# ZJU-FAST-Lab/uneven_planner

Measured on AMD Instinct MI355X. Metric: MINCO traj-opts/sec (batch), higher is better.
Workload: dtype f64

## Files before the change

### include/uneven_hip.h

```cpp
#ifndef UNEVEN_HIP_H
#define UNEVEN_HIP_H

#include <stdint.h>

#ifdef __cplusplus
extern "C" {
#endif

typedef struct uph_map uph_map;
typedef struct uph_ctx uph_ctx;
typedef struct uph_kino uph_kino;

#define UPH_OK 0
#define UPH_ERR_INVALID (-1)
#define UPH_ERR_HIP (-2)
#define UPH_ERR_NO_DEVICE (-3)
#define UPH_ERR_LIMIT (-4)
#define UPH_ERR_NO_CACHE (-5)

#define UPH_RET_STOPPED 3
#define UPH_RET_UNSUPPORTED 4

#define UPH_RET_LEFT_TILE 5
#define UPH_TILE_MARGIN 2.0
// ... 174 lines not shown
int uph_kino_stats(uph_kino* k, double* kernel_ms);

#define UPH_PLAN_PATH_CAP 1024
int uph_plan_upload(uph_kino* k, uph_ctx* c, const uph_manager_params* mp, int32_t B, const double* starts, const double* goals, int32_t path_cap,
                    int32_t* status, int32_t* traj_of, int32_t* n_inner_xy, int32_t* n_inner_yaw);
int uph_replan_upload(uph_kino* k, uph_ctx* src, uph_ctx* dst, const uph_manager_params* mp, int32_t B, const int32_t* src_traj, const double* t_switch,
                      const double* goals, int32_t path_cap, double* switch_states, int32_t* status, int32_t* traj_of, int32_t* n_inner_xy, int32_t* n_inner_yaw);
int uph_traj_states(uph_ctx* c, int32_t n, const int32_t* traj, const double* t, double* out10);
#define UPH_REFINE_AT_END 7
int uph_refine_upload(uph_ctx* src, uph_ctx* dst, int32_t B, const int32_t* src_traj, const double* t_switch, double* switch_states ,
                      int32_t* status, int32_t* traj_of, int32_t* n_inner_xy, int32_t* n_inner_yaw);
int uph_plan_staged(uph_ctx* c, int32_t cap_xy, int32_t cap_yaw, double* init_xy, double* end_xy, double* init_yaw, double* end_yaw, double* inner_xy,
                    double* inner_yaw, int32_t* n_inner_xy, int32_t* n_inner_yaw, double* total_time);

int uph_ctx_create(uph_map* m, const uph_opt_params* p, uph_ctx** out);
void uph_ctx_destroy(uph_ctx* c);
int uph_ctx_set_lanes(uph_ctx* c, int32_t lanes);
int uph_ctx_set_xcd_locality(uph_ctx* c, int32_t group);
int uph_ctx_set_wps(uph_ctx* c, int32_t wps);
int uph_ctx_set_sample_precision(uph_ctx* c, int32_t bits);
int uph_ctx_set_rho(uph_ctx* c, double rho);
int uph_ctx_get_rho(uph_ctx* c, double* rho);
int uph_ctx_set_trial_abandon(uph_ctx* c, int32_t on);

int uph_ctx_set_trace(uph_ctx* c, int32_t cap);
int uph_ctx_get_trace(uph_ctx* c, double* out);

int uph_optimize_batch(uph_ctx* c, int32_t B, const uph_problem* probs, uph_result* results);
int uph_optimize_batch_multi(uph_ctx* const* ctxs, int32_t n_gpus, int32_t B, const uph_problem* probs, uph_result* results);
int uph_multi_batch_plan(int32_t n_gpus, int32_t B, const uph_problem* probs, int32_t* share_of, double* predicted_cost);
int uph_batch_count(const uph_ctx* c);
int uph_batch_origin(const uph_ctx* c, int32_t* idx);
int uph_batch_upload(uph_ctx* c, int32_t B, const uph_problem* probs);
int uph_batch_solve(uph_ctx* c);
int uph_batch_solve_async(uph_ctx* c);
int uph_batch_wait(uph_ctx* c);
int uph_batch_download(uph_ctx* c, uph_result* results);
int uph_batch_stats(uph_ctx* c, double* kernel_ms, int64_t* evals, int64_t* sample_evals, int64_t* lbfgs_iters, int64_t* hist_bytes);
int uph_batch_abandon_stats(uph_ctx* c, int64_t* out5);

int uph_batch_prepare_ms(uph_ctx* c, double* ms);

int uph_batch_cycles(uph_ctx* c, long long* out);

int uph_eval_batch(uph_ctx* c, const double* x_packed, double* f, double* grad_packed, int32_t repeat);
int uph_penalty_batch(uph_ctx* c, int32_t repeat, int32_t store_residuals, double* cost, double* gdcxy_packed, double* gdcyaw_packed, double* gdT2);
// ... 67 lines not shown
```

### uneven_planner_amd/_lib.py

```python
import ctypes as C
import os

_HERE = os.path.dirname(os.path.abspath(__file__))
LIB_PATH = os.environ.get("UNEVENHIP_LIB") or os.path.join(_HERE, "libunevenhip.so")


class MapParams(C.Structure):
    _fields_ = [("iter_num", C.c_int32), ("map_size_x", C.c_double), ("map_size_y", C.c_double),
                ("ellipsoid_x", C.c_double), ("ellipsoid_y", C.c_double), ("ellipsoid_z", C.c_double),
                ("xy_resolution", C.c_double), ("yaw_resolution", C.c_double), ("min_cnormal", C.c_double),
                ("max_rho", C.c_double), ("gravity", C.c_double)]


class OptParams(C.Structure):
    _fields_ = [("rho_T", C.c_double), ("rho_ter", C.c_double), ("max_vel", C.c_double), ("max_acc_lon", C.c_double),
                ("max_acc_lat", C.c_double), ("max_kap", C.c_double), ("min_cxi", C.c_double), ("max_sig", C.c_double),
                ("use_scaling", C.c_int32), ("rho", C.c_double), ("beta", C.c_double), ("gamma", C.c_double),
                ("epsilon_con", C.c_double), ("max_iter", C.c_double), ("g_epsilon", C.c_double),
                ("min_step", C.c_double), ("inner_max_iter", C.c_double), ("delta", C.c_double),
                ("mem_size", C.c_int32), ("past", C.c_int32), ("int_K", C.c_int32)]


class ManagerParams(C.Structure):
    _fields_ = [("piece_len", C.c_double), ("mean_vel", C.c_double), ("init_time_times", C.c_double), ("yaw_piece_times", C.c_double),
# ... 78 lines not shown
    "uph_batch_count": (C.c_int, [_VP]),
    "uph_batch_origin": (C.c_int, [_VP, C.POINTER(_I32)]),
    "uph_map_cells_device": (C.c_int, [_VP, C.POINTER(_VP), C.POINTER(_I64)]),
    "uph_map_commit": (C.c_int, [_VP]),
    "uph_map_export_slab_dev": (C.c_int, [_VP, _I32, _I32, _VP]),
    "uph_map_import_cells_dev": (C.c_int, [_VP, _VP]),
    "uph_terrain_query": (C.c_int, [_VP, DP, _I32, DP, DP]),
    "uph_frontend_query": (C.c_int, [_VP, DP, _I32, DP, C.POINTER(C.c_int32), C.POINTER(C.c_int32)]),
    "uph_terrain_pose_query": (C.c_int, [_VP, DP, _I32, DP]),
    "uph_frontend_query_ms": (C.c_int, [_VP, DP]),
    "uph_map_filter_cloud": (_I64, [C.POINTER(C.c_float), _I64, C.POINTER(C.c_float), _I64]),
    "uph_map_build_stats": (C.c_int, [_VP, DP, C.POINTER(_I64), C.POINTER(_I64)]),
    "uph_map_build_stages": (C.c_int, [_VP, DP]),
    "uph_map_built_cloud": (_I64, [_VP, C.POINTER(C.c_float), _I64]),
    "uph_ctx_create": (C.c_int, [_VP, C.POINTER(OptParams), C.POINTER(_VP)]),
    "uph_ctx_destroy": (None, [_VP]),
    "uph_ctx_set_lanes": (C.c_int, [_VP, _I32]),
    "uph_ctx_set_wps": (C.c_int, [_VP, _I32]),
    "uph_ctx_set_xcd_locality": (C.c_int, [_VP, _I32]),
    "uph_ctx_set_sample_precision": (C.c_int, [_VP, _I32]),
    "uph_ctx_set_rho": (C.c_int, [_VP, C.c_double]),
    "uph_ctx_get_rho": (C.c_int, [_VP, DP]),
    "uph_ctx_set_trial_abandon": (C.c_int, [_VP, _I32]),
    "uph_ctx_set_trace": (C.c_int, [_VP, _I32]),
    "uph_ctx_get_trace": (C.c_int, [_VP, DP]),
    "uph_optimize_batch": (C.c_int, [_VP, _I32, C.POINTER(Problem), C.POINTER(Result)]),
    "uph_batch_upload": (C.c_int, [_VP, _I32, C.POINTER(Problem)]),
    "uph_batch_solve": (C.c_int, [_VP]),
    "uph_batch_solve_async": (C.c_int, [_VP]),
    "uph_batch_wait": (C.c_int, [_VP]),
    "uph_batch_download": (C.c_int, [_VP, C.POINTER(Result)]),
    "uph_batch_stats": (C.c_int, [_VP, DP, C.POINTER(_I64), C.POINTER(_I64), C.POINTER(_I64), C.POINTER(_I64)]),
    "uph_batch_prepare_ms": (C.c_int, [_VP, DP]),
    "uph_batch_abandon_stats": (C.c_int, [_VP, C.POINTER(_I64)]),
    "uph_batch_cycles": (C.c_int, [_VP, C.POINTER(C.c_longlong)]),
    "uph_build_id": (C.c_char_p, []),
    "uph_eval_batch": (C.c_int, [_VP, DP, DP, DP, _I32]),
    "uph_penalty_batch": (C.c_int, [_VP, _I32, _I32, DP, DP, DP, DP]),
    "uph_init_scaling_batch": (C.c_int, [_VP]),
    "uph_microbench_batch": (C.c_int, [_VP, _I32]),
    "uph_batch_set_state": (C.c_int, [_VP, DP, DP, DP, DP, DP]),
    "uph_report_batch": (C.c_int, [_VP, DP]),
    "uph_rollout_sizes": (C.c_int, [_I32, C.POINTER(_I32), DP, C.POINTER(_I32), DP, C.c_double, _I32, C.POINTER(_I64)]),
    "uph_rollout_plan": (C.c_int, [_VP, C.c_double, _I32, C.POINTER(_I64)]),
    "uph_rollout_batch": (C.c_int, [_VP, C.c_double, _I32, _I32, _I32, _I32, DP]),
    "uph_rollout_batch_dev": (C.c_int, [_VP, C.c_double, _I32, _I32, _I32, _I32, _VP]),
# ... 120 lines not shown
```

### uneven_planner_amd/alm_traj_opt.py

```python
import ctypes as C

import numpy as np

from . import _lib

HILL_OPT_PARAMS = dict(rho_T=100000.0, rho_ter=10.0, max_vel=0.5, max_acc_lon=5.0, max_acc_lat=10.0, max_kap=2.1,
                       min_cxi=0.8, max_sig=0.05, use_scaling=True, rho=1.0, beta=1000.0, gamma=1.0,
                       epsilon_con=0.001, max_iter=10.0, g_epsilon=1.0e-3, min_step=1.0e-32, inner_max_iter=10000.0,
                       delta=1.0e-4, mem_size=256, past=3, int_K=16)
_INT_FIELDS = ("use_scaling", "mem_size", "past", "int_K")


def pack_problems(probs, int_K=16, with_sizes=False):
    arr = (_lib.Problem * len(probs))()
    keep, sizes = [], []
    for i, pr in enumerate(probs):
        ixy = np.ascontiguousarray(np.asarray(pr["inner_xy"], dtype=np.float64).T)
        iyw = np.ascontiguousarray(pr["inner_yaw"], dtype=np.float64)
        keep += [ixy, iyw]
        a = arr[i]
        a.n_inner_xy, a.n_inner_yaw = ixy.shape[0], iyw.shape[0]
        a.init_xy[:] = np.asarray(pr["init_xy"], dtype=np.float64).T.ravel().tolist()
        a.end_xy[:] = np.asarray(pr["end_xy"], dtype=np.float64).T.ravel().tolist()
        a.init_yaw[:] = np.asarray(pr["init_yaw"], dtype=np.float64).ravel().tolist()
# ... 411 lines not shown
            self.h = None
        p = _lib.OptParams(**{k: (int(getattr(self, k)) if k in _INT_FIELDS else float(getattr(self, k))) for k in self._pnames})
        h = C.c_void_p()
        _lib.check(self.L.uph_ctx_create(env.h, C.byref(p), C.byref(h)), "uph_ctx_create")
        self.h = h

    def set_lanes(self, lanes):
        _lib.check(self.L.uph_ctx_set_lanes(self.h, int(lanes)), "uph_ctx_set_lanes")

    def set_xcd_locality(self, group):
        _lib.check(self.L.uph_ctx_set_xcd_locality(self.h, int(group)), "uph_ctx_set_xcd_locality")

    def set_wps(self, wps):
        _lib.check(self.L.uph_ctx_set_wps(self.h, int(wps)), "uph_ctx_set_wps")

    def set_sample_precision(self, bits):
        _lib.check(self.L.uph_ctx_set_sample_precision(self.h, int(bits)), "uph_ctx_set_sample_precision")

    def set_rho(self, rho):
        _lib.check(self.L.uph_ctx_set_rho(self.h, float(rho)), "uph_ctx_set_rho")

    def set_trial_abandon(self, on):
        _lib.check(self.L.uph_ctx_set_trial_abandon(self.h, 1 if on else 0), "uph_ctx_set_trial_abandon")

    def get_rho(self):
        r = C.c_double(0)
        _lib.check(self.L.uph_ctx_get_rho(self.h, C.byref(r)), "uph_ctx_get_rho")
        return r.value

    def _make_problems(self, probs):
        arr, keep, self._sizes = pack_problems(probs, int(self.int_K), with_sizes=True)
        return arr, keep

    def upload(self, probs):
        arr, keep = self._make_problems(probs)
        self._B = 0
        _lib.check(self.L.uph_batch_upload(self.h, len(probs), arr), "uph_batch_upload")
        self._B = len(probs)
        self._trace_cap_up = getattr(self, "_trace_cap", 0)

    def solve(self):
        _lib.check(self.L.uph_batch_solve(self.h), "uph_batch_solve")

    def solve_async(self):
        _lib.check(self.L.uph_batch_solve_async(self.h), "uph_batch_solve_async")

# ... 529 lines not shown
```

### uneven_planner_amd/csrc/solver_program.hpp

```cpp
#pragma once
#include "terrain_dev.hpp"
#include "trajectory_dev.hpp"
#include "uph_common.hpp"

namespace uph {

#ifndef UPH_GRID_FROM_MEM
#define UPH_GRID_FROM_MEM 1
#endif
#ifndef UPH_PHASE_MASK
#define UPH_PHASE_MASK 15
#endif
#ifndef UPH_STATE_PROBE
#define UPH_STATE_PROBE(st) do { } while (0)
#endif
#ifndef UPH_SCALING_WB
#define UPH_SCALING_WB 8
#endif
#ifndef UPH_SC_XB
#define UPH_SC_XB 9
#endif
#ifndef UPH_SC_YB
#define UPH_SC_YB 14
#endif
#ifndef UPH_SC_WLO
#define UPH_SC_WLO 2
#endif
#ifndef UPH_SC_WHI
#define UPH_SC_WHI 3
#endif

#ifndef UPH_ASIDE_PREP
#define UPH_ASIDE_PREP 1
#endif
template <class WG, class F>
UPH_HD void asideKnotSolve(WG& wg, int lenW, int lenX, int n, F f) {
    (void)lenW; (void)lenX;
    wg.pfor(n, f);
}

template <class WG, class SR = double>
struct Solver {
    WG& wg;
    const GridDev& grid;
    const OptParams& P;
    const BatchDev& bd;
    const TrajDesc& td;
    int Nxy, Nyaw, n, S, K, mem, CH, CHP, recd;
    int CHS;
    int* rtag;
    double *x, *xp, *g, *gp, *d, *cxy, *cyaw, *Gxy, *Gyaw, *gamxy, *gamyaw, *bt, *rec, *wtab, *ttab, *pf, *hd;
    double* ab;
    int* abn;
    static constexpr int AB_DOUBLES = 4;
    double* up;
    static constexpr int UP_DOUBLES = 6;
    UPH_HD void tally(int k, bool yes) {
#if defined(__HIP_DEVICE_COMPILE__)
        if (yes && wg.wave == 0) abn[k] = abn[k] + 1;
#else
        if (yes) abn[k]++;
#endif
// ... 802 lines not shown

    UPH_HD void initScaling(double* x0) {
        generate<false>(x0, 0.0);
        const double tau = x0[0];
        const double dTau = getTtoTauGrad(tau);
        double js[3];
        expand(x0, 1.0, js);
        double sm[3] = {0.0, 0.0, 0.0};
        for (int s0 = 0; s0 < S; s0 += CHS) {
            const int cnt = S - s0 < CHS ? S - s0 : CHS;
            double part[3];
            wg.template sum<3>(cnt, part, [&](int t, double* acc) { sampleObjective(s0 + t, t, acc); });
            sm[0] += part[0]; sm[1] += part[1]; sm[2] += part[2];
            scatterChunk(s0, cnt);
        }
        double chx, chy;
        adjoint(chx, chy);
        const double gTau_fx = (P.rho_T + (js[1] + sm[1] + chx) / Nxy + (js[2] + sm[2] + chy) / Nyaw) * dTau;
        const double mq = wg.maxv((Nxy - 1) * 2 + (Nyaw - 1), [&](int t) {
            return t < (Nxy - 1) * 2 ? fabs(gamxy[3 * 2 + t]) : fabs(gamyaw[3 + (t - (Nxy - 1) * 2)]);
        });
        scale_fx = wg.bcast(1.0 / dmax(1.0, dmax(mq, fabs(gTau_fx))));
        wg.pfor(2, [&](int u) { fillTimes(u); });
        wg.pfor(S, [&](int s) { scalingSample(s, dTau); });
    }

    UPH_HD void scalingSample(int s, double dTau) {
        const int i = divSmall(s, K + 1, inv_k1), j = s - i * (K + 1);
        Kin k;
        kin(i, j, k);
#if !defined(UPH_SCALING_GROUPS) || UPH_SCALING_GROUPS == 2
        scalingGroup<0, 4>(s, i, j, k, dTau);
        scalingGroup<4, 3>(s, i, j, k, dTau);
#elif UPH_SCALING_GROUPS == 3
        scalingGroup<0, 3>(s, i, j, k, dTau);
        scalingGroup<3, 2>(s, i, j, k, dTau);
        scalingGroup<5, 2>(s, i, j, k, dTau);
#else
        scalingGroup<0, 7>(s, i, j, k, dTau);
#endif
    }
    template <int Q0, int NQS>
    UPH_HD void scalingGroup(int s, int i, int j, const Kin& k, double dTau) {
        const int nbx = Nxy + 5, nby = Nyaw + 5;
        const double Tx = Txy, Ty = Tyaw, itx = 1.0 / Txy, ity = 1.0 / Tyaw;
        const double gravity = grid.gravity;
        const double alpha = 1.0 / K * j;
        const double icvx = k.tv[0], icvy = k.tv[2], icxi = k.tv[5];
        const int m = k.yaw_idx;
        double dpL[NQS][2], dvL[NQS][2], daL[NQS][2], dpR[NQS][2], dvR[NQS][2], daR[NQS][2];
        double ypL[NQS], yvL[NQS], yaL[NQS], ypR[NQS], yvR[NQS], yaR[NQS];
        double sumx[NQS], sumy[NQS], mx[NQS];
#pragma unroll
        for (int qi = 0; qi < NQS; qi++) {
            const int q = Q0 + qi;
            double gp_[2] = {0, 0}, gv_[2] = {0, 0}, ga_[2] = {0, 0}, gyaw = 0.0, gdyaw = 0.0, gse2[3];
            if (q == 0) {
                gv_[0] = k.syaw; gv_[1] = -k.cyaw;
                gyaw = k.vel[0] * k.cyaw + k.vel[1] * k.syaw;
            } else if (q == 1) {
                for (int t = 0; t < 2; t++) gv_[t] = 1.0 * icvx * icvx * 2.0 * k.vel[t];
                for (int t = 0; t < 3; t++) gse2[t] = 1.0 * k.v_norm * k.v_norm * 2.0 * icvx * k.tg[0][t];
                gp_[0] = gse2[0]; gp_[1] = gse2[1]; gyaw = gse2[2];
            } else if (q == 2) {
                const double gax = 2.0 * k.ax;
                ga_[0] = gax * icvx * k.cyaw; ga_[1] = gax * icvx * k.syaw;
                gyaw = gax * icvx * k.lat_acc;
// ... 31 lines not shown
                chain_y += -(double)kk * cyaw[6 * m + kk] * ity * vy;
                gy_[kk] = vy * sy;
                sx *= itx; sy *= ity;
            }
            double tx = ((gp_[0] * k.vel[0] + gp_[1] * k.vel[1]) + (gv_[0] * k.acc[0] + gv_[1] * k.acc[1]) + (ga_[0] * k.jer[0] + ga_[1] * k.jer[1])) * alpha;
            const double yawdot = gyaw * k.dyaw + gdyaw * k.d2yaw;
            tx += yawdot * (alpha + i);
            const double ty = -yawdot * m;
            sumx[qi] = tx + chain_x;
            sumy[qi] = ty + chain_y;
            mx[qi] = 0.0;
            for (int t = 0; t < 2; t++) {
                const double g0 = gx_[0][t], g1 = gx_[1][t], g2 = gx_[2][t], g3 = gx_[3][t], g4 = gx_[4][t], g5 = gx_[5][t];
                dpL[qi][t] = g0 - 10.0 * g3 + 15.0 * g4 - 6.0 * g5; dvL[qi][t] = g1 - 6.0 * g3 + 8.0 * g4 - 3.0 * g5; daL[qi][t] = 0.5 * g2 - 1.5 * g3 + 1.5 * g4 - 0.5 * g5;
                dpR[qi][t] = 10.0 * g3 - 15.0 * g4 + 6.0 * g5; dvR[qi][t] = -4.0 * g3 + 7.0 * g4 - 3.0 * g5; daR[qi][t] = 0.5 * g3 - g4 + 0.5 * g5;
            }
            {
                const double g0 = gy_[0], g1 = gy_[1], g2 = gy_[2], g3 = gy_[3], g4 = gy_[4], g5 = gy_[5];
                ypL[qi] = g0 - 10.0 * g3 + 15.0 * g4 - 6.0 * g5; yvL[qi] = g1 - 6.0 * g3 + 8.0 * g4 - 3.0 * g5; yaL[qi] = 0.5 * g2 - 1.5 * g3 + 1.5 * g4 - 0.5 * g5;
                ypR[qi] = 10.0 * g3 - 15.0 * g4 + 6.0 * g5; yvR[qi] = -4.0 * g3 + 7.0 * g4 - 3.0 * g5; yaR[qi] = 0.5 * g3 - g4 + 0.5 * g5;
            }
        }
        const bool inL = i >= 1, inR = i + 1 <= Nxy - 1;
        const auto WL = UPH_AS_GLOBAL(Wr_xy + (size_t)(inL ? 2 * (i - 1) : 0) * nbx);
        const auto WR = UPH_AS_GLOBAL(Wr_xy + (size_t)(inR ? 2 * i : 0) * nbx);
        const int pcL = knotCol(i, Nxy), pcR = knotCol(i + 1, Nxy);
        for (int c0 = 3; c0 < Nxy + 2; c0 += UPH_SCALING_WB) {
            double w[4][UPH_SCALING_WB];
#pragma unroll
            for (int u = 0; u < UPH_SCALING_WB; u++) {
                const int cc = c0 + u < Nxy + 2 ? c0 + u : Nxy + 1;
                w[0][u] = WL[cc]; w[1][u] = WL[nbx + cc]; w[2][u] = WR[cc]; w[3][u] = WR[nbx + cc];
            }
#pragma unroll
            for (int q = 0; q < NQS; q++) {
                const double c00 = inL ? dvL[q][0] : 0.0, c01 = inL ? dvL[q][1] : 0.0, c10 = inL ? daL[q][0] : 0.0, c11 = inL ? daL[q][1] : 0.0;
                const double c20 = inR ? dvR[q][0] : 0.0, c21 = inR ? dvR[q][1] : 0.0, c30 = inR ? daR[q][0] : 0.0, c31 = inR ? daR[q][1] : 0.0;
                double mq = mx[q];
#pragma unroll
                for (int u = 0; u < UPH_SCALING_WB; u++) {
                    const int col = c0 + u;
                    double a0 = (w[0][u] * c00 + w[1][u] * c10) + (w[2][u] * c20 + w[3][u] * c30);
                    double a1 = (w[0][u] * c01 + w[1][u] * c11) + (w[2][u] * c21 + w[3][u] * c31);
                    if (col == pcL) { a0 += dpL[q][0]; a1 += dpL[q][1]; }
                    if (col == pcR) { a0 += dpR[q][0]; a1 += dpR[q][1]; }
                    if (col < Nxy + 2) mq = dmax(mq, dmax(fabs(a0), fabs(a1)));
                }
                mx[q] = mq;
            }
        }
        double htx[NQS], hty[NQS];
        {
            const int sc[4] = {1, 2, Nxy + 3, Nxy + 4};
            double w[4][4];
#pragma unroll
            for (int u = 0; u < 4; u++) { w[0][u] = WL[sc[u]]; w[1][u] = WL[nbx + sc[u]]; w[2][u] = WR[sc[u]]; w[3][u] = WR[nbx + sc[u]]; }
#pragma unroll
            for (int q = 0; q < NQS; q++) {
                const double c00 = inL ? dvL[q][0] : 0.0, c01 = inL ? dvL[q][1] : 0.0, c10 = inL ? daL[q][0] : 0.0, c11 = inL ? daL[q][1] : 0.0;
                const double c20 = inR ? dvR[q][0] : 0.0, c21 = inR ? dvR[q][1] : 0.0, c30 = inR ? daR[q][0] : 0.0, c31 = inR ? daR[q][1] : 0.0;
                double a0[4], a1[4];
#pragma unroll
                for (int u = 0; u < 4; u++) {
                    a0[u] = (w[0][u] * c00 + w[1][u] * c10) + (w[2][u] * c20 + w[3][u] * c30);
                    a1[u] = (w[0][u] * c01 + w[1][u] * c11) + (w[2][u] * c21 + w[3][u] * c31);
                }
                if (!inL) { a0[0] += dvL[q][0]; a1[0] += dvL[q][1]; a0[1] += daL[q][0]; a1[1] += daL[q][1]; }
                if (!inR) { a0[2] += dvR[q][0]; a1[2] += dvR[q][1]; a0[3] += daR[q][0]; a1[3] += daR[q][1]; }
                double headtail_x = 0.0;
                headtail_x += a0[0] * hd[2] + a1[0] * hd[3];
                headtail_x += 2.0 * Tx * (a0[1] * hd[4] + a1[1] * hd[5]);
                headtail_x += a0[2] * hd[8] + a1[2] * hd[9];
                headtail_x += 2.0 * Tx * (a0[3] * hd[10] + a1[3] * hd[11]);
                htx[q] = headtail_x;
            }
        }
        const bool yL = m >= 1, yR = m + 1 <= Nyaw - 1;
        const auto VL = UPH_AS_GLOBAL(Wr_yaw + (size_t)(yL ? 2 * (m - 1) : 0) * nby);
        const auto VR = UPH_AS_GLOBAL(Wr_yaw + (size_t)(yR ? 2 * m : 0) * nby);
        const int qL = knotCol(m, Nyaw), qR = knotCol(m + 1, Nyaw);
        for (int c0 = 3; c0 < Nyaw + 2; c0 += UPH_SCALING_WB) {
            double w[4][UPH_SCALING_WB];
#pragma unroll
            for (int u = 0; u < UPH_SCALING_WB; u++) {
                const int cc = c0 + u < Nyaw + 2 ? c0 + u : Nyaw + 1;
                w[0][u] = VL[cc]; w[1][u] = VL[nby + cc]; w[2][u] = VR[cc]; w[3][u] = VR[nby + cc];
            }
#pragma unroll
            for (int q = 0; q < NQS; q++) {
                const double y0_ = yL ? yvL[q] : 0.0, y1_ = yL ? yaL[q] : 0.0, y2_ = yR ? yvR[q] : 0.0, y3_ = yR ? yaR[q] : 0.0;
                double mq = mx[q];
#pragma unroll
                for (int u = 0; u < UPH_SCALING_WB; u++) {
                    const int col = c0 + u;
                    double a0 = (w[0][u] * y0_ + w[1][u] * y1_) + (w[2][u] * y2_ + w[3][u] * y3_);
                    if (col == qL) a0 += ypL[q];
                    if (col == qR) a0 += ypR[q];
                    if (col < Nyaw + 2) mq = dmax(mq, fabs(a0));
                }
                mx[q] = mq;
            }
        }
        {
            const int sc[4] = {1, 2, Nyaw + 3, Nyaw + 4};
            double w[4][4];
#pragma unroll
            for (int u = 0; u < 4; u++) { w[0][u] = VL[sc[u]]; w[1][u] = VL[nby + sc[u]]; w[2][u] = VR[sc[u]]; w[3][u] = VR[nby + sc[u]]; }
#pragma unroll
            for (int q = 0; q < NQS; q++) {
                const double y0_ = yL ? yvL[q] : 0.0, y1_ = yL ? yaL[q] : 0.0, y2_ = yR ? yvR[q] : 0.0, y3_ = yR ? yaR[q] : 0.0;
                double a0[4];
#pragma unroll
                for (int u = 0; u < 4; u++) a0[u] = (w[0][u] * y0_ + w[1][u] * y1_) + (w[2][u] * y2_ + w[3][u] * y3_);
                if (!yL) { a0[0] += yvL[q]; a0[1] += yaL[q]; }
                if (!yR) { a0[2] += yvR[q]; a0[3] += yaR[q]; }
                double headtail_y = 0.0;
// ... 453 lines not shown
```

### uneven_planner_amd/csrc/unevenhip.hip

```cpp
#include <hip/hip_runtime.h>

#include <type_traits>

#include <algorithm>
#include <cmath>
#include <cstdio>
#include <cstdlib>
#include <cstring>
#include <map>
#include <numeric>
#include <string>
#include <thread>
#include <vector>

#include "../../include/uneven_hip.h"
#include "minco_op_host.hpp"
#include "resample_walk.hpp"
#include "solver_program.hpp"
#include "uph_ctx.hpp"
#include "wave_dev.hpp"

using namespace uph;

#ifndef UPH_THOMAS_KPL
// ... 453 lines not shown
            else twoLoopT<8, 2>(d, g, dg_out, al_lds, n, hist, m, end, bound, scale);
            __builtin_amdgcn_s_setprio(0);
        }
        bar(1);
    }
    template <class F>
    __device__ __forceinline__ double maxv(int n, F f) {
        double a = 0.0;
        for (int i = ftid(); i < n; i += NT) { const double v = f(i); a = v > a ? v : a; }
        a = waveMax(a);
        double* r = red + par * (NW * MAXM);
        par ^= 1;
        if (lane == 0) r[wave * MAXM] = a;
        bar(0);
        double t = r[0];
#pragma unroll
        for (int w = 1; w < NW; w++) t = r[w * MAXM] > t ? r[w * MAXM] : t;
        return uni(t);
    }
};

template <int NT, class F>
__device__ __forceinline__ void asideKnotSolve(DevWG<NT>& wg, int lenW, int lenX, int n, F f) { wg.aside(lenW, lenX, n, f); }

template <int NT, int WPS, int MODE, bool F32S = false>
__global__ __launch_bounds__(NT, WPS) void uph_solver_kernel(GridDev grid, OptParams P, BatchDev bd, int repeat) {
    extern __shared__ double lds[];
    const int w = blockIdx.x;
    if (w >= bd.B) return;
    const int b = bd.order ? bd.order[w] : w;
    DevWG<NT> wg(lds);
    typedef typename std::conditional<F32S, f32r, double>::type SR;
    Solver<DevWG<NT>, SR> sol(wg, grid, P, bd, b, lds + DevWG<NT>::SCRATCH);
    TrajState& st = bd.state[b];
    if (MODE == 0) sol.evalOnly(st, repeat);
    else if (MODE == 1) sol.prepare(st);
    else if (MODE == 2) sol.optimize(st, repeat);
    else if (MODE == 7) sol.resumeHook(st, repeat >> 1, repeat & 1);
    else if (MODE == 8) { if (repeat & 1) sol.template penaltyOnly<true>(st, repeat >> 1); else sol.template penaltyOnly<false>(st, repeat >> 1); }
    else if (MODE == 3) sol.report(st);
    else if (MODE == 5) sol.microbench(st, repeat);
    else sol.scalingOnly(st);
}

__global__ void uph_fill_kernel(double* __restrict__ p, size_t n, double v) {
    for (size_t i = (size_t)blockIdx.x * blockDim.x + threadIdx.x; i < n; i += (size_t)gridDim.x * blockDim.x) p[i] = v;
// ... 218 lines not shown
            HIPCHK(hipMemcpyAsync(c->d_gridmem.p, c->grid_host_framed.data(), sizeof(GridDev) * c->frames.size(), hipMemcpyHostToDevice, c->stream));
            c->framed_from = grid;
            c->framed_valid = true;
        }
    }
    return UPH_OK;
}

int refreshStates(uph_ctx* c) {
    HIPCHK(hipMemcpy(c->state_host.data(), c->d_state.p, sizeof(TrajState) * c->B, hipMemcpyDeviceToHost));
    return UPH_OK;
}

static int launchSolver(uph_ctx* c, int mode, int repeat, bool async = false, hipEvent_t evb = nullptr, hipEvent_t eve = nullptr) {
    if (!async && c->pending) { setError("an asynchronous solve is in flight on this context: call uph_batch_wait first"); return UPH_ERR_INVALID; }
    if (!evb) { evb = c->ev0; eve = c->ev1; }
    HIPCHK(hipSetDevice(uphMapDevice(c->map)));
    GridDev grid;
    const int rg = syncGridMem(c, grid);
    if (rg != UPH_OK) return rg;
    if (c->d_parammem.ensure(sizeof(OptParams))) return UPH_ERR_HIP;
    HIPCHK(hipMemcpyAsync(c->d_parammem.p, &c->P, sizeof(OptParams), hipMemcpyHostToDevice, c->stream));
    BatchDev bd = makeBatchDev(c);
#define UPH_LAUNCH(NTL, WPS, MODE)                                                                                                     \
    do {                                                                                                                             \
        const size_t ldsmax = 160 * 1024;    \
        HIPCHK(hipFuncSetAttribute((const void*)uph_solver_kernel<NTL, WPS, MODE>, hipFuncAttributeMaxDynamicSharedMemorySize, (int)ldsmax)); \
        HIPCHK(hipEventRecord(evb, c->stream));                                                                                   \
        BatchDev bm = bd;                                                                                                            \
        bm.B = c->n_main;                                                                                                            \
        if (c->n_main < c->B) {            \
            BatchDev bb = bd;              \
            bb.B = c->B - c->n_main;                                                                                                 \
            bb.order = bd.order + c->n_main;                                                                                         \
            HIPCHK(hipStreamWaitEvent(c->stream2, evb, 0));                                                                       \
            hipLaunchKernelGGL((uph_solver_kernel<NTL, WPS, MODE>), dim3(bb.B), dim3(NTL), c->lds_big, c->stream2, grid, c->P, bb, repeat); \
            HIPCHK(hipEventRecord(c->ev2, c->stream2));                                                                              \
        }                                                                                                                            \
        hipLaunchKernelGGL((uph_solver_kernel<NTL, WPS, MODE>), dim3(c->n_main), dim3(NTL), c->lds_bytes, c->stream, grid, c->P, bm, repeat); \
        if (c->n_main < c->B) HIPCHK(hipStreamWaitEvent(c->stream, c->ev2, 0));                                                      \
    } while (0)
#define UPH_LAUNCH_MODE(NTL, WPS)                                                                                                      \
    do {                                                                                                                             \
        if (mode == 0) UPH_LAUNCH(NTL, WPS, 0);                                                                                      \
        else if (mode == 1) UPH_LAUNCH(NTL, WPS, 1);                                                                                 \
        else if (mode == 2) UPH_LAUNCH(NTL, WPS, 2);                                                                                 \
        else if (mode == 3) UPH_LAUNCH(NTL, WPS, 3);                                                                                 \
        else if (mode == 5) UPH_LAUNCH(NTL, WPS, 5);                                                                                 \
        else UPH_LAUNCH(NTL, WPS, 4);                                                                                                \
    } while (0)
#define UPH_LAUNCH32(NTL, WPS, MODE)                                                                                                   \
    do {                                                                                                                             \
        const size_t ldsmax = 160 * 1024;    \
        HIPCHK(hipFuncSetAttribute((const void*)uph_solver_kernel<NTL, WPS, MODE, true>, hipFuncAttributeMaxDynamicSharedMemorySize, (int)ldsmax)); \
        HIPCHK(hipEventRecord(evb, c->stream));                                                                                   \
        BatchDev bm = bd;                                                                                                            \
        bm.B = c->n_main;                                                                                                            \
        if (c->n_main < c->B) {                                                                                                      \
            BatchDev bb = bd;                                                                                                        \
            bb.B = c->B - c->n_main;                                                                                                 \
            bb.order = bd.order + c->n_main;                                                                                         \
            HIPCHK(hipStreamWaitEvent(c->stream2, evb, 0));                                                                       \
// ... 119 lines not shown
    if (c->ev0) hipEventDestroy(c->ev0);
    if (c->ev1) hipEventDestroy(c->ev1);
    if (c->stream) hipStreamDestroy(c->stream);
    if (c->stream2) hipStreamDestroy(c->stream2);
    if (c->ev2) hipEventDestroy(c->ev2);
    if (c->evp0) hipEventDestroy(c->evp0);
    if (c->evp1) hipEventDestroy(c->evp1);
    delete c;
}

int uph_ctx_set_lanes(uph_ctx* c, int32_t lanes) {
    if (!c || (lanes != 0 && lanes != 64 && lanes != 128 && lanes != 256 && lanes != 512)) return UPH_ERR_INVALID;
    c->lanes_forced = lanes;
    return UPH_OK;
}
int uph_ctx_set_xcd_locality(uph_ctx* c, int32_t group) { if (!c || group < 0) return UPH_ERR_INVALID; c->xcd_group = group; return UPH_OK; }
int uph_ctx_set_wps(uph_ctx* c, int32_t wps) { if (!c || wps < 0 || wps > 2) return UPH_ERR_INVALID; c->wps_forced = wps; return UPH_OK; }
int uph_ctx_set_sample_precision(uph_ctx* c, int32_t bits) {
    if (!c || (bits != 32 && bits != 64)) { setError("uph_ctx_set_sample_precision: 32 or 64"); return UPH_ERR_INVALID; }
    c->sample_f32 = bits == 32;
    return UPH_OK;
}
int uph_ctx_set_rho(uph_ctx* c, double rho) { if (!c) return UPH_ERR_INVALID; c->rho = rho; return UPH_OK; }
int uph_ctx_set_trial_abandon(uph_ctx* c, int32_t on) { if (!c || (on != 0 && on != 1)) return UPH_ERR_INVALID; c->P.no_trial_abandon = on ? 0 : 1; return UPH_OK; }
int uph_ctx_get_rho(uph_ctx* c, double* rho) { if (!c || !rho) return UPH_ERR_INVALID; *rho = c->rho; return UPH_OK; }

int uph_ctx_set_trace(uph_ctx* c, int32_t cap) { if (!c || cap < 0) return UPH_ERR_INVALID; c->trace_cap = cap; return UPH_OK; }
int uph_ctx_get_trace(uph_ctx* c, double* out ) {
    if (c && c->pending) { setError("an asynchronous solve is in flight on this context: call uph_batch_wait first"); return UPH_ERR_INVALID; }
    if (!c || !out || c->trace_cap_up <= 0 || c->B <= 0) return UPH_ERR_INVALID;
    HIPCHK(hipSetDevice(uphMapDevice(c->map)));
    HIPCHK(hipMemcpy(out, c->d_trace.p, sizeof(double) * (size_t)c->B * c->trace_cap_up, hipMemcpyDeviceToHost));
    return UPH_OK;
}

static void yawTurnKink(const uph_problem& pr, double& turn, double& kink) {
    double prev = pr.init_yaw[0];
    turn = 0.0; kink = 0.0;
    for (int i = 0; i <= pr.n_inner_yaw; i++) {
        const double cur = i < pr.n_inner_yaw ? pr.inner_yaw[i] : pr.end_yaw[0];
        const double dy = std::fabs(cur - prev);
        turn += dy; kink = std::max(kink, dy); prev = cur;
    }
}
static double predictedCostOf(int32_t n_inner_xy, int32_t n_inner_yaw, double turn, double kink) {
    const double n = 2.0 * n_inner_xy + n_inner_yaw + 1.0;
// ... 139 lines not shown
            const int G = c->xcd_group & ~7;
            for (int g0 = 0; g0 + G <= B; g0 += G) {
                std::vector<int> bins[8], spill, placed((size_t)G, -1);
                for (int k = 0; k < G; k++) bins[octant(c->order[g0 + k])].push_back(c->order[g0 + k]);
                for (int r = 0; r < 8; r++) {
                    int at = r;
                    for (int b : bins[r]) { if (at < G) { placed[at] = b; at += 8; } else spill.push_back(b); }
                }
                size_t sp = 0;
                for (int k = 0; k < G; k++) if (placed[k] < 0) placed[k] = spill[sp++];
                for (int k = 0; k < G; k++) c->order[g0 + k] = placed[k];
            }
        }
        const size_t limit = c->lanes == 128 ? 40960 : (c->lanes == 256 ? 81920 : (c->lanes == 512 ? 163840 : 32768));
        c->n_main = B; c->lds_big = 0;
        size_t mmain = 0, mbig = 0;
        int nbig = 0;
        for (int b = 0; b < B; b++) { if (c->fp_bytes[b] > limit) { nbig++; mbig = std::max(mbig, c->fp_bytes[b]); } else mmain = std::max(mmain, c->fp_bytes[b]); }
        if (nbig > 0 && nbig < B) {
            std::stable_partition(c->order.begin(), c->order.end(), [&](int a) { return c->fp_bytes[a] <= limit; });
            c->n_main = B - nbig; c->lds_bytes = mmain; c->lds_big = mbig;
        }
    }
    c->state_host.assign(B, TrajState());
    for (int b = 0; b < B; b++) { std::memset(&c->state_host[b], 0, sizeof(TrajState)); c->state_host[b].rho = c->rho; c->state_host[b].scale_fx = 1.0; }
    return UPH_OK;
}

static int commitBatch(uph_ctx* c, int32_t B) {
    HIPCHK(hipMemcpyAsync(c->d_desc.p, c->desc.data(), sizeof(TrajDesc) * B, hipMemcpyHostToDevice, c->stream));
    HIPCHK(hipMemcpyAsync(c->d_order.p, c->order.data(), 4 * B, hipMemcpyHostToDevice, c->stream));
    HIPCHK(hipMemcpyAsync(c->d_state.p, c->state_host.data(), sizeof(TrajState) * B, hipMemcpyHostToDevice, c->stream));
    HIPCHK(hipMemsetAsync(c->d_hist.p, 0, 8 * c->sum_hist, c->stream));
    HIPCHK(hipMemsetAsync(c->d_dual.p, 0, 8 * 7 * c->sum_S, c->stream));
    HIPCHK(hipMemsetAsync(c->d_res.p, 0, 8 * 7 * c->sum_S, c->stream));
    hipLaunchKernelGGL(uph_fill_kernel, dim3(1024), dim3(256), 0, c->stream, c->d_scl.as<double>(), (size_t)7 * c->sum_S, 1.0);
    HIPCHK(hipGetLastError());
    if (c->trace_cap > 0) HIPCHK(hipMemsetAsync(c->d_trace.p, 0, 8 * (size_t)c->trace_cap * B, c->stream));
    HIPCHK(hipStreamSynchronize(c->stream));
    c->trace_cap_up = c->trace_cap;
    c->B = B;
    return UPH_OK;
}

int uph_batch_upload(uph_ctx* c, int32_t B, const uph_problem* probs) {
    if (!c || B <= 0 || !probs) { setError("uph_batch_upload: bad arguments"); return UPH_ERR_INVALID; }
// ... 736 lines not shown
```

### uneven_planner_amd/csrc/uph_common.hpp

```cpp
#pragma once
#include <math.h>
#include <stdint.h>

#if defined(__HIPCC__)
#define UPH_HD __host__ __device__ __forceinline__
#define UPH_NOINLINE __host__ __device__ __attribute__((noinline))
#else
#define UPH_HD inline
#define UPH_NOINLINE __attribute__((noinline))
#endif

#if defined(__HIP_DEVICE_COMPILE__)
#define UPH_AS_GLOBAL(p) ((const __attribute__((address_space(1))) double*)(p))
#else
#define UPH_AS_GLOBAL(p) (p)
#endif

#if defined(UPH_ISA_MARKS) && defined(__HIP_DEVICE_COMPILE__)
#define UPH_MARK(name) asm volatile("; UPHMARK " name)
#else
#define UPH_MARK(name) do { } while (0)
#endif

namespace uph {
// ... 113 lines not shown
    const MincoOp* ops;
    const double* x0;
    double* x;
    double* gout;
    double* dual;
    double* res;
    double* scl;
    double* cxy;
    double* cyaw;
    double* hist;
    double* rs_d;
    double* rs;
    double* report;
    double* pen_gxy;
    double* pen_gyaw;
    double* pen_out;
    double* trace;
    int trace_cap;
    const int* order;
    const OptParams* params_mem;
    const GridDev* grid_mem;
    int grid_per_traj;
    const double* thomas;
};

#if defined(__HIP_DEVICE_COMPILE__)
UPH_HD void pinv(double& v) { asm volatile("" : "+v"(v)); }
UPH_HD void pinv(float& v) { asm volatile("" : "+v"(v)); }
UPH_HD void pinv(int& v) { asm volatile("" : "+v"(v)); }
#else
UPH_HD void pinv(double&) {}
UPH_HD void pinv(float&) {}
UPH_HD void pinv(int&) {}
#endif
#ifndef UPH_DIET
#define UPH_DIET 0
#endif

UPH_HD double dmax(double a, double b) { return a > b ? a : b; }
UPH_HD double dmin(double a, double b) { return a < b ? a : b; }

UPH_HD double expC2(double tau) { return tau > 0.0 ? ((0.5 * tau + 1.0) * tau + 1.0) : 1.0 / ((0.5 * tau - 1.0) * tau + 1.0); }
UPH_HD double divR(double x, double y, double r) {
    const double q0 = x * r;
    return fma(fma(-q0, y, x), r, q0);
}
UPH_HD void mv2(const double* M, double v0, double v1, double& o0, double& o1) {
// ... 141 lines not shown
```

### uneven_planner_amd/csrc/uph_ctx.hpp

```cpp
#pragma once
#include <hip/hip_runtime.h>

#include <map>
#include <string>
#include <vector>

#include "uph_internal.hpp"

using namespace uph;

struct DevBuf {
    void* p = nullptr;
    size_t cap = 0;
    int ensure(size_t bytes) {
        if (bytes <= cap) return 0;
        if (p) hipFree(p);
        p = nullptr; cap = 0;
        size_t want = bytes + bytes / 4 + 256;
        if (hipMalloc(&p, want) != hipSuccess) { setError("hipMalloc failed"); return -1; }
        cap = want;
        return 0;
    }
    void release() { if (p) hipFree(p); p = nullptr; cap = 0; }
    template <class T> T* as() { return (T*)p; }
// ... 22 lines not shown
    double init_xy[6], end_xy[6], init_yaw[3], end_yaw[3], total_time = 0.0;
    double lo[2], hi[2];
    double turn = 0.0, kink = 0.0;
};
struct uph_ctx {
    uph_map* map = nullptr;
    int device = 0;
    OptParams P;
    double rho = 1.0;
    hipStream_t stream = nullptr;
    hipEvent_t ev0 = nullptr, ev1 = nullptr;
    std::map<int, int> op_index;
    std::vector<MincoOp> ops_host;
    std::vector<void*> op_allocs;
    DevBuf d_ops;
    bool ops_dirty = false;
    int B = 0;
    std::vector<TrajDesc> desc;
    std::vector<int> order;
    int64_t sum_n = 0, sum_S = 0, sum_cxy = 0, sum_cyaw = 0, sum_hist = 0;
    size_t lds_bytes = 0;
    size_t lds_big = 0;
    int n_main = 0;
    std::vector<int> rejected;
    int n_rejected = 0;
    bool all_rejected = false;
    std::vector<TrajFrame> frames;
    std::vector<GridDev> grid_host_framed;
    GridDev frames_grid;
    GridDev framed_from;
    bool framed_valid = false;
    std::vector<int> origin;
    bool sample_f32 = false;
    int xcd_group = 0;
    hipStream_t stream2 = nullptr;
    hipEvent_t evp0 = nullptr, evp1 = nullptr;
    bool pending = false;
    hipEvent_t ev2 = nullptr;
    std::vector<size_t> fp_bytes;
    int lanes = 64;
    int lanes_forced = 0;
    int wps = 1;
    int wps_forced = 0;
    DevBuf d_thomas, d_rsd, d_rs, d_gridmem, d_parammem;
    GridDev grid_host;
    DevBuf d_desc, d_state, d_x, d_x0, d_gout, d_dual, d_res, d_scl, d_cxy, d_cyaw, d_hist, d_report, d_order, d_trace;
// ... 47 lines not shown
```

Measured before the change: 54330.

## Stage scaling-sample knot weight rows into LDS per chunk

During the scaling initialization stage, each chunk of samples first copies the band of Wr_xy/Wr_yaw knot rows it needs from global memory into spare LDS, then reads the weights from LDS with a smaller unroll width. This targets repeated global loads of the same weight rows across lanes. It is on by default for the main launch in modes 1 and 4, but it enlarges dynamic LDS per block, which may lower occupancy. It also adds per-chunk reductions and a copy step, and falls back to the global path when the band does not fit.

Result: no change. 54490 (median of 6 runs) (+0.3%).

```diff
diff --git a/include/uneven_hip.h b/include/uneven_hip.h
--- a/include/uneven_hip.h
+++ b/include/uneven_hip.h
@@ -220,6 +220,7 @@
 int uph_ctx_set_rho(uph_ctx* c, double rho);
 int uph_ctx_get_rho(uph_ctx* c, double* rho);
 int uph_ctx_set_trial_abandon(uph_ctx* c, int32_t on);
+int uph_ctx_set_scaling_stage(uph_ctx* c, int32_t on);
 
 int uph_ctx_set_trace(uph_ctx* c, int32_t cap);
 int uph_ctx_get_trace(uph_ctx* c, double* out);
diff --git a/uneven_planner_amd/_lib.py b/uneven_planner_amd/_lib.py
--- a/uneven_planner_amd/_lib.py
+++ b/uneven_planner_amd/_lib.py
@@ -124,6 +124,7 @@
     "uph_ctx_set_rho": (C.c_int, [_VP, C.c_double]),
     "uph_ctx_get_rho": (C.c_int, [_VP, DP]),
     "uph_ctx_set_trial_abandon": (C.c_int, [_VP, _I32]),
+    "uph_ctx_set_scaling_stage": (C.c_int, [_VP, _I32]),
     "uph_ctx_set_trace": (C.c_int, [_VP, _I32]),
     "uph_ctx_get_trace": (C.c_int, [_VP, DP]),
     "uph_optimize_batch": (C.c_int, [_VP, _I32, C.POINTER(Problem), C.POINTER(Result)]),
diff --git a/uneven_planner_amd/alm_traj_opt.py b/uneven_planner_amd/alm_traj_opt.py
--- a/uneven_planner_amd/alm_traj_opt.py
+++ b/uneven_planner_amd/alm_traj_opt.py
@@ -457,6 +457,9 @@
 
     def set_trial_abandon(self, on):
         _lib.check(self.L.uph_ctx_set_trial_abandon(self.h, 1 if on else 0), "uph_ctx_set_trial_abandon")
+
+    def set_scaling_stage(self, on):
+        _lib.check(self.L.uph_ctx_set_scaling_stage(self.h, 1 if on else 0), "uph_ctx_set_scaling_stage")
 
     def get_rho(self):
         r = C.c_double(0)
diff --git a/uneven_planner_amd/csrc/solver_program.hpp b/uneven_planner_amd/csrc/solver_program.hpp
--- a/uneven_planner_amd/csrc/solver_program.hpp
+++ b/uneven_planner_amd/csrc/solver_program.hpp
@@ -1,4 +1,7 @@
 #pragma once
+#if defined(UPH_STAGE_ASSERT) && !defined(__HIP_DEVICE_COMPILE__)
+#include <assert.h>
+#endif
 #include "terrain_dev.hpp"
 #include "trajectory_dev.hpp"
 #include "uph_common.hpp"
@@ -16,6 +19,14 @@
 #endif
 #ifndef UPH_SCALING_WB
 #define UPH_SCALING_WB 8
+#endif
+#ifndef UPH_SCALING_WB_LDS
+#define UPH_SCALING_WB_LDS 4
+#endif
+#if defined(UPH_STAGE_ASSERT) && !defined(__HIP_DEVICE_COMPILE__)
+#define UPH_STAGE_CHECK(cond) assert(cond)
+#else
+#define UPH_STAGE_CHECK(cond) do { } while (0)
 #endif
 #ifndef UPH_SC_XB
 #define UPH_SC_XB 9
@@ -38,6 +49,21 @@
     (void)lenW; (void)lenX;
     wg.pfor(n, f);
 }
+
+template <class WG, class SOL>
+UPH_HD bool scalingRoundsStaged(WG& wg, SOL& sol, double dTau) {
+    (void)wg;
+#if defined(UPH_HOST_STAGE_DOUBLES) && !defined(__HIP_DEVICE_COMPILE__)
+    double* stage = new double[UPH_HOST_STAGE_DOUBLES + 2];
+    sol.scalingStaged(dTau, stage, UPH_HOST_STAGE_DOUBLES);
+    delete[] stage;
+    return true;
+#else
+    (void)sol; (void)dTau;
+    return false;
+#endif
+}
+struct alignas(16) StageWord { double a, b; };
 
 template <class WG, class SR = double>
 struct Solver {
@@ -886,27 +912,79 @@
         });
         scale_fx = wg.bcast(1.0 / dmax(1.0, dmax(mq, fabs(gTau_fx))));
         wg.pfor(2, [&](int u) { fillTimes(u); });
-        wg.pfor(S, [&](int s) { scalingSample(s, dTau); });
-    }
-
+        if (!scalingRoundsStaged(wg, *this, dTau)) wg.pfor(S, [&](int s) { scalingSample(s, dTau); });
+    }
+
+    int sg_kx = 1, sg_ky = 1, sg_nky = 1, sg_yoff = 0;
+    const double* sg_base = nullptr;
+    UPH_HD int yawPieceOf(int s) const {
+        const int i = divSmall(s, K + 1, inv_k1), j = s - i * (K + 1);
+        const double s1 = bt[Nxy + 1 + j];
+        const double now_time = s1 + bt[i];
+        int yi = toInt<double>(divR(now_time, double(Tyaw), double(ec_iTyaw)));
+        if (yi >= Nyaw) yi = Nyaw - 1;
+        if (yi < 0) yi = 0;
+        return yi;
+    }
+    UPH_HD void scalingStaged(double dTau, double* stg, int cap) {
+        const int nbx = Nxy + 5, nby = Nyaw + 5, CHR = wg.size();
+        sg_base = stg;
+        for (int s0 = 0; s0 < S; s0 += CHR) {
+            const int cnt = S - s0 < CHR ? S - s0 : CHR;
+            int kx = 1, nkx = 0, ky = 1, nky = 0;
+            if (cap > 0) {
+                const int i0 = divSmall(s0, K + 1, inv_k1), i1 = divSmall(s0 + cnt - 1, K + 1, inv_k1);
+                const int mhi = (int)wg.maxv(cnt, [&](int t) { return (double)yawPieceOf(s0 + t); });
+                const int mlo = Nyaw - 1 - (int)wg.maxv(cnt, [&](int t) { return (double)(Nyaw - 1 - yawPieceOf(s0 + t)); });
+                stagedKnots(i0, i1, Nxy, kx, nkx);
+                stagedKnots(mlo - 1, mhi + 1, Nyaw, ky, nky);
+            }
+            const int lenx = 2 * nkx * nbx, leny = 2 * nky * nby;
+            if (cap <= 0 || lenx + leny > cap) {
+                wg.pfor(cnt, [&](int t) { scalingSample<false>(s0 + t, dTau); });
+                continue;
+            }
+            sg_kx = kx; sg_ky = ky; sg_nky = nky; sg_yoff = lenx;
+            const double* srcx = Wr_xy + (size_t)(2 * (kx - 1)) * nbx;
+            const double* srcy = Wr_yaw + (size_t)(2 * (ky - 1)) * nby;
+            wg.pfor((lenx + leny) >> 1, [&](int t) {
+                const int tx = lenx >> 1;
+#if defined(__HIP_DEVICE_COMPILE__)
+                typedef const __attribute__((address_space(1))) StageWord* src_t;
+#else
+                typedef const StageWord* src_t;
+#endif
+                ((StageWord*)stg)[t] = t < tx ? ((src_t)(const void*)srcx)[t] : ((src_t)(const void*)srcy)[t - tx];
+            });
+            wg.pfor(cnt, [&](int t) { scalingSample<true>(s0 + t, dTau); });
+        }
+    }
+
+    template <bool STG = false>
     UPH_HD void scalingSample(int s, double dTau) {
         const int i = divSmall(s, K + 1, inv_k1), j = s - i * (K + 1);
         Kin k;
         kin(i, j, k);
 #if !defined(UPH_SCALING_GROUPS) || UPH_SCALING_GROUPS == 2
-        scalingGroup<0, 4>(s, i, j, k, dTau);
-        scalingGroup<4, 3>(s, i, j, k, dTau);
+        scalingGroup<0, 4, STG>(s, i, j, k, dTau);
+        scalingGroup<4, 3, STG>(s, i, j, k, dTau);
 #elif UPH_SCALING_GROUPS == 3
-        scalingGroup<0, 3>(s, i, j, k, dTau);
-        scalingGroup<3, 2>(s, i, j, k, dTau);
-        scalingGroup<5, 2>(s, i, j, k, dTau);
+        scalingGroup<0, 3, STG>(s, i, j, k, dTau);
+        scalingGroup<3, 2, STG>(s, i, j, k, dTau);
+        scalingGroup<5, 2, STG>(s, i, j, k, dTau);
 #else
-        scalingGroup<0, 7>(s, i, j, k, dTau);
-#endif
-    }
-    template <int Q0, int NQS>
+        scalingGroup<0, 7, STG>(s, i, j, k, dTau);
+#endif
+    }
+    template <bool STG>
+    UPH_HD auto knotRows(const double* W, const double* staged, int knot, int knot0, int nb) const {
+        if constexpr (STG) return staged + (size_t)(2 * (knot - knot0)) * nb;
+        else return UPH_AS_GLOBAL(W + (size_t)(2 * (knot - 1)) * nb);
+    }
+    template <int Q0, int NQS, bool STG>
     UPH_HD void scalingGroup(int s, int i, int j, const Kin& k, double dTau) {
         const int nbx = Nxy + 5, nby = Nyaw + 5;
+        constexpr int WB = STG ? UPH_SCALING_WB_LDS : UPH_SCALING_WB;
         const double Tx = Txy, Ty = Tyaw, itx = 1.0 / Txy, ity = 1.0 / Tyaw;
         const double gravity = grid.gravity;
         const double alpha = 1.0 / K * j;
@@ -984,13 +1062,14 @@
             }
         }
         const bool inL = i >= 1, inR = i + 1 <= Nxy - 1;
-        const auto WL = UPH_AS_GLOBAL(Wr_xy + (size_t)(inL ? 2 * (i - 1) : 0) * nbx);
-        const auto WR = UPH_AS_GLOBAL(Wr_xy + (size_t)(inR ? 2 * i : 0) * nbx);
+        const int kxe = STG ? sg_kx : 1;
+        const auto WL = knotRows<STG>(Wr_xy, sg_base, inL ? i : kxe, sg_kx, nbx);
+        const auto WR = knotRows<STG>(Wr_xy, sg_base, inR ? i + 1 : kxe, sg_kx, nbx);
         const int pcL = knotCol(i, Nxy), pcR = knotCol(i + 1, Nxy);
-        for (int c0 = 3; c0 < Nxy + 2; c0 += UPH_SCALING_WB) {
-            double w[4][UPH_SCALING_WB];
-#pragma unroll
-            for (int u = 0; u < UPH_SCALING_WB; u++) {
+        for (int c0 = 3; c0 < Nxy + 2; c0 += WB) {
+            double w[4][WB];
+#pragma unroll
+            for (int u = 0; u < WB; u++) {
                 const int cc = c0 + u < Nxy + 2 ? c0 + u : Nxy + 1;
                 w[0][u] = WL[cc]; w[1][u] = WL[nbx + cc]; w[2][u] = WR[cc]; w[3][u] = WR[nbx + cc];
             }
@@ -1000,7 +1079,7 @@
                 const double c20 = inR ? dvR[q][0] : 0.0, c21 = inR ? dvR[q][1] : 0.0, c30 = inR ? daR[q][0] : 0.0, c31 = inR ? daR[q][1] : 0.0;
                 double mq = mx[q];
 #pragma unroll
-                for (int u = 0; u < UPH_SCALING_WB; u++) {
+                for (int u = 0; u < WB; u++) {
                     const int col = c0 + u;
                     double a0 = (w[0][u] * c00 + w[1][u] * c10) + (w[2][u] * c20 + w[3][u] * c30);
                     double a1 = (w[0][u] * c01 + w[1][u] * c11) + (w[2][u] * c21 + w[3][u] * c31);
@@ -1038,13 +1117,20 @@
             }
         }
         const bool yL = m >= 1, yR = m + 1 <= Nyaw - 1;
-        const auto VL = UPH_AS_GLOBAL(Wr_yaw + (size_t)(yL ? 2 * (m - 1) : 0) * nby);
-        const auto VR = UPH_AS_GLOBAL(Wr_yaw + (size_t)(yR ? 2 * m : 0) * nby);
+        const int kye = STG ? sg_ky : 1;
+        int kyl = yL ? m : kye, kyr = yR ? m + 1 : kye;
+        if (STG) {
+            UPH_STAGE_CHECK(kyl >= sg_ky && kyl < sg_ky + sg_nky && kyr >= sg_ky && kyr < sg_ky + sg_nky);
+            kyl = kyl < sg_ky ? sg_ky : (kyl > sg_ky + sg_nky - 1 ? sg_ky + sg_nky - 1 : kyl);
+            kyr = kyr < sg_ky ? sg_ky : (kyr > sg_ky + sg_nky - 1 ? sg_ky + sg_nky - 1 : kyr);
+        }
+        const auto VL = knotRows<STG>(Wr_yaw, sg_base + sg_yoff, kyl, sg_ky, nby);
+        const auto VR = knotRows<STG>(Wr_yaw, sg_base + sg_yoff, kyr, sg_ky, nby);
         const int qL = knotCol(m, Nyaw), qR = knotCol(m + 1, Nyaw);
-        for (int c0 = 3; c0 < Nyaw + 2; c0 += UPH_SCALING_WB) {
-            double w[4][UPH_SCALING_WB];
-#pragma unroll
-            for (int u = 0; u < UPH_SCALING_WB; u++) {
+        for (int c0 = 3; c0 < Nyaw + 2; c0 += WB) {
+            double w[4][WB];
+#pragma unroll
+            for (int u = 0; u < WB; u++) {
                 const int cc = c0 + u < Nyaw + 2 ? c0 + u : Nyaw + 1;
                 w[0][u] = VL[cc]; w[1][u] = VL[nby + cc]; w[2][u] = VR[cc]; w[3][u] = VR[nby + cc];
             }
@@ -1053,7 +1139,7 @@
                 const double y0_ = yL ? yvL[q] : 0.0, y1_ = yL ? yaL[q] : 0.0, y2_ = yR ? yvR[q] : 0.0, y3_ = yR ? yaR[q] : 0.0;
                 double mq = mx[q];
 #pragma unroll
-                for (int u = 0; u < UPH_SCALING_WB; u++) {
+                for (int u = 0; u < WB; u++) {
                     const int col = c0 + u;
                     double a0 = (w[0][u] * y0_ + w[1][u] * y1_) + (w[2][u] * y2_ + w[3][u] * y3_);
                     if (col == qL) a0 += ypL[q];
diff --git a/uneven_planner_amd/csrc/unevenhip.hip b/uneven_planner_amd/csrc/unevenhip.hip
--- a/uneven_planner_amd/csrc/unevenhip.hip
+++ b/uneven_planner_amd/csrc/unevenhip.hip
@@ -499,6 +499,13 @@
 
 template <int NT, class F>
 __device__ __forceinline__ void asideKnotSolve(DevWG<NT>& wg, int lenW, int lenX, int n, F f) { wg.aside(lenW, lenX, n, f); }
+
+template <int NT, class SOL>
+__device__ __forceinline__ bool scalingRoundsStaged(DevWG<NT>& wg, SOL& sol, double dTau) {
+    (void)wg;
+    sol.scalingStaged(dTau, sol.x + sol.bd.stage_off, sol.bd.stage_cap);
+    return true;
+}
 
 template <int NT, int WPS, int MODE, bool F32S = false>
 __global__ __launch_bounds__(NT, WPS) void uph_solver_kernel(GridDev grid, OptParams P, BatchDev bd, int repeat) {
@@ -763,6 +770,17 @@
     if (c->d_parammem.ensure(sizeof(OptParams))) return UPH_ERR_HIP;
     HIPCHK(hipMemcpyAsync(c->d_parammem.p, &c->P, sizeof(OptParams), hipMemcpyHostToDevice, c->stream));
     BatchDev bd = makeBatchDev(c);
+    size_t lds_main = c->lds_bytes;
+    if ((mode == 1 || mode == 4) && c->scaling_stage && c->stage_want > 0) {
+        const size_t budget = c->lanes == 64 ? 40 * 1024 : (c->lanes == 128 ? 80 * 1024 : 160 * 1024);
+        const size_t base = (c->lds_bytes + 15) & ~(size_t)15;
+        if (base + 4096 <= budget) {
+            const size_t cap = std::min(c->stage_want, budget - base);
+            bd.stage_off = (int)(base / 8) - DevWG<64>::MAXM * 2 * (c->lanes / 64);
+            bd.stage_cap = (int)(cap / 8);
+            lds_main = base + cap;
+        }
+    }
 #define UPH_LAUNCH(NTL, WPS, MODE)                                                                                                     \
     do {                                                                                                                             \
         const size_t ldsmax = 160 * 1024;    \
@@ -773,12 +791,13 @@
         if (c->n_main < c->B) {            \
             BatchDev bb = bd;              \
             bb.B = c->B - c->n_main;                                                                                                 \
+            bb.stage_off = bb.stage_cap = 0;                                                                                         \
             bb.order = bd.order + c->n_main;                                                                                         \
             HIPCHK(hipStreamWaitEvent(c->stream2, evb, 0));                                                                       \
             hipLaunchKernelGGL((uph_solver_kernel<NTL, WPS, MODE>), dim3(bb.B), dim3(NTL), c->lds_big, c->stream2, grid, c->P, bb, repeat); \
             HIPCHK(hipEventRecord(c->ev2, c->stream2));                                                                              \
         }                                                                                                                            \
-        hipLaunchKernelGGL((uph_solver_kernel<NTL, WPS, MODE>), dim3(c->n_main), dim3(NTL), c->lds_bytes, c->stream, grid, c->P, bm, repeat); \
+        hipLaunchKernelGGL((uph_solver_kernel<NTL, WPS, MODE>), dim3(c->n_main), dim3(NTL), lds_main, c->stream, grid, c->P, bm, repeat); \
         if (c->n_main < c->B) HIPCHK(hipStreamWaitEvent(c->stream, c->ev2, 0));                                                      \
     } while (0)
 #define UPH_LAUNCH_MODE(NTL, WPS)                                                                                                      \
@@ -944,6 +963,7 @@
     return UPH_OK;
 }
 int uph_ctx_set_rho(uph_ctx* c, double rho) { if (!c) return UPH_ERR_INVALID; c->rho = rho; return UPH_OK; }
+int uph_ctx_set_scaling_stage(uph_ctx* c, int32_t on) { if (!c || (on != 0 && on != 1)) return UPH_ERR_INVALID; c->scaling_stage = on != 0; return UPH_OK; }
 int uph_ctx_set_trial_abandon(uph_ctx* c, int32_t on) { if (!c || (on != 0 && on != 1)) return UPH_ERR_INVALID; c->P.no_trial_abandon = on ? 0 : 1; return UPH_OK; }
 int uph_ctx_get_rho(uph_ctx* c, double* rho) { if (!c || !rho) return UPH_ERR_INVALID; *rho = c->rho; return UPH_OK; }
 
@@ -1129,6 +1149,11 @@
             c->n_main = B - nbig; c->lds_bytes = mmain; c->lds_big = mbig;
         }
     }
+    c->stage_want = 0;
+    for (int k = 0; k < c->n_main; k++) {
+        const TrajDesc& t = c->desc[c->order[k]];
+        c->stage_want = std::max(c->stage_want, scalingStageBytes(t.Nxy, t.Nyaw, c->P.int_K, c->lanes));
+    }
     c->state_host.assign(B, TrajState());
     for (int b = 0; b < B; b++) { std::memset(&c->state_host[b], 0, sizeof(TrajState)); c->state_host[b].rho = c->rho; c->state_host[b].scale_fx = 1.0; }
     return UPH_OK;
diff --git a/uneven_planner_amd/csrc/uph_common.hpp b/uneven_planner_amd/csrc/uph_common.hpp
--- a/uneven_planner_amd/csrc/uph_common.hpp
+++ b/uneven_planner_amd/csrc/uph_common.hpp
@@ -159,7 +159,27 @@
     const GridDev* grid_mem;
     int grid_per_traj;
     const double* thomas;
-};
+    int stage_off, stage_cap;
+};
+
+UPH_HD void stagedKnots(int p0, int p1, int N, int& k0, int& nk) {
+    k0 = p0 < 1 ? 1 : (p0 > N - 1 ? N - 1 : p0);
+    if (k0 < 1) k0 = 1;
+    int k1 = p1 + 1 > N - 1 ? N - 1 : p1 + 1;
+    if (k1 < k0) k1 = k0;
+    nk = k1 - k0 + 1;
+}
+inline size_t scalingStageBytes(int Nxy, int Nyaw, int K, int lanes) {
+    int px = (lanes - 1) / (K + 1) + 2;
+    if (px > Nxy) px = Nxy;
+    int py = (int)((long long)px * Nyaw / Nxy) + 4;
+    if (py > Nyaw) py = Nyaw;
+    int nkx = px + 1, nky = py + 3;
+    const int mx = Nxy - 1 < 1 ? 1 : Nxy - 1, my = Nyaw - 1 < 1 ? 1 : Nyaw - 1;
+    if (nkx > mx) nkx = mx;
+    if (nky > my) nky = my;
+    return (size_t)16 * ((size_t)nkx * (Nxy + 5) + (size_t)nky * (Nyaw + 5));
+}
 
 #if defined(__HIP_DEVICE_COMPILE__)
 UPH_HD void pinv(double& v) { asm volatile("" : "+v"(v)); }
diff --git a/uneven_planner_amd/csrc/uph_ctx.hpp b/uneven_planner_amd/csrc/uph_ctx.hpp
--- a/uneven_planner_amd/csrc/uph_ctx.hpp
+++ b/uneven_planner_amd/csrc/uph_ctx.hpp
@@ -68,6 +68,8 @@
     size_t lds_bytes = 0;
     size_t lds_big = 0;
     int n_main = 0;
+    bool scaling_stage = true;
+    size_t stage_want = 0;
     std::vector<int> rejected;
     int n_rejected = 0;
     bool all_rejected = false;
```
